# Wuziyi616/CFUN

Hardware: AMD Instinct MI355X
Metric: volumes/sec fwd+bwd, 256x256x128 8-class CT (higher is better)
Workload: dtype f32; 1 GPU; cfg2: 256x256x128 CT, stage 'finetune', 4 positive + 8 negative RoIs, U-Net b=20, 96x96x96 crops -> 192x192x192 masks, 6 losses incl. 3-D Sobel edge loss, fwd+bwd; parallelism=single GPU

## Files before the change

cfun_amd/_lib.py:

```python
import ctypes as C
import os

import torch

_HERE = os.path.dirname(os.path.abspath(__file__))
DEFAULT_LIB = os.path.join(_HERE, "libcfun_hip.so")

ACT_NONE, ACT_RELU, ACT_LRELU = 0, 1, 2
ALGO_AUTO, ALGO_DIRECT, ALGO_MFMA = 0, 1, 2
ALGO_WINO = 4
ALGO_WINO2 = 5
TILE_G16, TILE_G8 = 0x100, 0x200


class ConvParams(C.Structure):
    _fields_ = [(n, C.c_int32) for n in ("N", "Di", "Hi", "Wi", "Ci", "Do", "Ho", "Wo", "Co", "CoP", "CiP",
                                         "kd", "kh", "kw", "stride", "pd", "ph", "pw", "up2", "act")] + \
               [("slope", C.c_float)] + \
               [(n, C.c_int32) for n in ("scale_mode", "has_shift", "res_mode", "res_up2", "d2s", "d2s_cq", "tap_skip", "algo",
                                         "w_prepared")]


class ConvFusion(C.Structure):
    _fields_ = [("in_stats", C.c_void_p), ("in_act", C.c_int32), ("in_slope", C.c_float), ("out_stats", C.c_void_p),
                ("out_eps", C.c_float)]


FUSE_OUT_STATS, FUSE_IN_NORM, FUSE_IN_NORM_WGRAD = 1, 2, 4


class WeightJob(C.Structure):
    _fields_ = [("w", C.c_void_p), ("fwd", C.c_void_p), ("dgrad", C.c_void_p), ("co_idx", C.c_void_p), ("ci_idx", C.c_void_p),
                ("Co", C.c_int32), ("Ci", C.c_int32), ("T", C.c_int32), ("src_ci", C.c_int32), ("fwd_kind", C.c_int32),
                ("dgrad_kind", C.c_int32), ("block_begin", C.c_uint32), ("reserved", C.c_int32)]


WOP_NONE = 0

_P = C.c_void_p
_I = C.c_int32
_L = C.c_int64
_F = C.c_float
_Z = C.c_size_t
_PP = C.POINTER(ConvParams)
_PF = C.POINTER(ConvFusion)
# ... 213 lines not shown
```

cfun_amd/csrc/common.h:

```cpp
#pragma once
#include <hip/hip_runtime.h>
#include <stdint.h>
#include <stdlib.h>

#include "../../include/cfun_hip.h"

#define CFUN_WAVE 64

#ifdef CFUN_HIP_EMULATION
#define CFUN_DYN_LDS(T, name) T* name = reinterpret_cast<T*>(hipemu::g.dyn_lds)
#else
#define CFUN_DYN_LDS(T, name) extern __shared__ __attribute__((aligned(16))) T name[]
#endif

#define CFUN_LAUNCH_CHECK()                         \
  do {                                              \
    hipError_t e__ = hipGetLastError();             \
    if (e__ != hipSuccess) return (int)e__;         \
  } while (0)

static inline hipStream_t cfun_st(cfun_stream_t s) { return (hipStream_t)s; }

static inline size_t cfun_align_up(size_t v, size_t a) { return (v + a - 1) / a * a; }

static inline bool cfun_aligned16(const void* p) { return (((uintptr_t)p) & 15) == 0; }

struct CfunWgradDst { float* ptr; int oidhw; };

__device__ __forceinline__ float cfun_apply_act(float v, int act, float slope) {
  if (act == CFUN_ACT_RELU) return v > 0.f ? v : 0.f;
  if (act == CFUN_ACT_LRELU) return v > 0.f ? v : v * slope;
  return v;
}

__device__ __forceinline__ float cfun_fast_sqrt(float v) {
#ifdef CFUN_HIP_EMULATION
  return sqrtf(v);
#else
  return __builtin_amdgcn_sqrtf(v);
#endif
}
__device__ __forceinline__ float cfun_fast_rcp(float v) {
#ifdef CFUN_HIP_EMULATION
  return 1.0f / v;
#else
  return __builtin_amdgcn_rcpf(v);
#endif
}

__device__ __forceinline__ float cfun_fast_rsq(float v) {
#ifdef CFUN_HIP_EMULATION
  return 1.0f / sqrtf(v);
#else
  return __builtin_amdgcn_rsqf(v);
#endif
}

__device__ __forceinline__ float cfun_wave_sum(float v) {
#pragma unroll
  for (int o = 32; o > 0; o >>= 1) v += __shfl_xor(v, o, 64);
  return v;
}
__device__ __forceinline__ double cfun_wave_sum_d(double v) {
#pragma unroll
  for (int o = 32; o > 0; o >>= 1) v += __shfl_xor(v, o, 64);
  return v;
}
// ... 1 lines not shown
```

cfun_amd/csrc/conv3d.hip:

```cpp
#include <stdlib.h>

#include "conv3d_mfma.h"
#include "../../include/cfun_tile.h"

int cfun_conv_fwd_direct(const float*, const float*, const float*, const float*, const float*, float*,
                         const CfunConv3dParams*, hipStream_t);
int cfun_conv_bwd_data_direct(const float*, const float*, float*, const CfunConv3dParams*, hipStream_t);
int cfun_conv_bwd_weight_direct(const float*, const float*, CfunWgradDst, const CfunConv3dParams*, void*, size_t, hipStream_t);
size_t cfun_direct_wgrad_ws(const CfunConv3dParams*);
int cfun_wgrad_finish(const float*, CfunWgradDst, const CfunConv3dParams*, int, hipStream_t);
int cfun_wgrad_zero(CfunWgradDst, const CfunConv3dParams*, hipStream_t);
int cfun_conv_stem_supported(const CfunConv3dParams*);
int cfun_conv_stem_fwd(const float*, const float*, const float*, const float*, float*, const CfunConv3dParams*, hipStream_t);
int cfun_conv_pointwise_supported(const CfunConv3dParams*);
int cfun_conv_pointwise_in_supported(const CfunConv3dParams*);
int cfun_conv_pointwise_fwd(const float*, const float*, const float*, const float*, const float*, float*,
                            const CfunConv3dParams*, const float*, int, float, hipStream_t);
int cfun_wino_supported(const CfunConv3dParams*);
size_t cfun_wino_workspace_bytes(const CfunConv3dParams*);
int cfun_wino_s2d_dgrad_supported(const CfunConv3dParams*, const CfunConv3dParams*);
int cfun_wino_fwd(const float*, const float*, int, int, const float*, const float*, const float*, float*,
                  const CfunConv3dParams*, void*, size_t, const cfun_mfma::ConvMode*, int, hipStream_t);
int cfun_wino_is_2d(const CfunConv3dParams*);
int cfun_wino_geom(const CfunConv3dParams*);
// ... 132 lines not shown
  if (q->pd < 0 || q->ph < 0 || q->pw < 0) return false;
  q->up2 = 0; q->act = CFUN_ACT_NONE; q->scale_mode = 0; q->has_shift = 0; q->res_mode = 0; q->res_up2 = 0;
  q->d2s = 0; q->d2s_cq = 0; q->tap_skip = 0; q->w_prepared = 0;
  return true;
}

bool use_folded_s2_dgrad(const CfunConv3dParams* p) {
  return CFUN_ALGO_OF(p->algo) != CFUN_ALGO_DIRECT && p->stride == 2 && !p->up2 && !p->d2s && p->kd == 3 && p->kh == 3 && p->kw == 3 &&
         p->pd == 1 && p->ph == 1 && p->pw == 1 && !((p->Di | p->Hi | p->Wi) & 1) && !(p->Ci & 3) && !(p->Co & 3) &&
         p->Di == 2 * p->Do && p->Hi == 2 * p->Ho && p->Wi == 2 * p->Wo;
}

__global__ void __launch_bounds__(256)
k_fold_s2_dgrad_weights(const float* __restrict__ wpT, float* __restrict__ wd, int Ci, int Co, int CiP, int CoPd) {
  const int64_t total = (int64_t)8 * Co * CoPd;
  const int64_t i = (int64_t)blockIdx.x * 256 + threadIdx.x;
  if (i >= total) return;
  const int col = (int)(i % CoPd);
  const int co = (int)((i / CoPd) % Co);
  const int tap = (int)(i / ((int64_t)CoPd * Co));
  float v = 0.f;
  if (col < 8 * Ci) {
    const int q = col / Ci, ci = col - q * Ci;
    const int par[3] = {q >> 2, (q >> 1) & 1, q & 1}, off[3] = {tap >> 2, (tap >> 1) & 1, tap & 1};
    int t[3];
    bool ok = true;
    for (int d = 0; d < 3; ++d) {
      if (par[d] == 0) { t[d] = 1; ok = ok && off[d] == 0; }
      else t[d] = off[d] == 0 ? 2 : 0;
    }
    if (ok) v = wpT[((int64_t)((t[0] * 3 + t[1]) * 3 + t[2]) * Co + co) * CiP + ci];
  }
  wd[i] = v;
}

CfunConv3dParams folded_s2_params(const CfunConv3dParams* p) {
  CfunConv3dParams q = *p;
  q.Di = p->Do; q.Hi = p->Ho; q.Wi = p->Wo; q.Ci = p->Co;
  q.Do = p->Do; q.Ho = p->Ho; q.Wo = p->Wo; q.Co = 8 * p->Ci;
  q.CoP = (8 * p->Ci + 15) / 16 * 16; q.CiP = p->CoP;
  q.kd = q.kh = q.kw = 2; q.stride = 1; q.pd = q.ph = q.pw = 0;
  q.up2 = 0; q.act = CFUN_ACT_NONE; q.scale_mode = 0; q.has_shift = 0; q.res_mode = 0; q.res_up2 = 0; q.d2s = 1;
  q.d2s_cq = 0; q.tap_skip = 0; q.w_prepared = 0;
  return q;
}

int wgrad_max_nsub(const Shape* s) {
  static int cap = -1;
  if (cap < 0) {
    const char* e = getenv("CFUN_WGRAD_MAX_NSUB");
    cap = e ? atoi(e) : 5;
    if (cap < 1 || cap > 5) cap = 5;
  }
  return s->max_nsub < cap ? s->max_nsub : cap;
}

int wgrad_nsub(const CfunConv3dParams* p, const Shape* s) {
  if (p->d2s && p->tap_skip) {
    const int cqp = p->Co >> 3, mx = wgrad_max_nsub(s);
    const int tiles = (cqp + 16 * mx - 1) / (16 * mx);
    return (cqp + 16 * tiles - 1) / (16 * tiles);
  }
  return pick_nsub(p->CoP, wgrad_max_nsub(s));
}

bool use_mfma_dgrad(const CfunConv3dParams* p, CfunConv3dParams* q, const Shape** s) {
// ... 106 lines not shown
  __syncthreads();
  if (vl == 0) {
    for (int l = 1; l < lanes; ++l) {
      const int t2 = l * C4 + cg;
#pragma unroll
      for (int q = 0; q < 2; ++q)
#pragma unroll
        for (int j = 0; j < 4; ++j) acc[q][j] += sm[(t2 * 2 + q) * 4 + j];
    }
    double* out = part + ((int64_t)n * gridDim.x + blockIdx.x) * 2 * p.Co;
#pragma unroll
    for (int q = 0; q < 2; ++q)
#pragma unroll
      for (int j = 0; j < 4; ++j) out[(int64_t)q * p.Co + co + j] = acc[q][j];
  }
}

int splitk_stats_blocks(const CfunConv3dParams* p, int* lanes_out) {
  const int C4 = p->Co >> 2;
  if ((p->Co & 3) || C4 > 256 || C4 < 1) return 0;
  const int lanes = 256 / C4;
  const int64_t V = (int64_t)p->Do * p->Ho * p->Wo;
  int64_t want = (4096 + p->N - 1) / (p->N > 0 ? p->N : 1);
  int64_t maxb = (V + (int64_t)lanes * 4 - 1) / ((int64_t)lanes * 4);
  if (maxb < 1) maxb = 1;
  if (lanes_out) *lanes_out = lanes;
  return (int)(want < maxb ? want : maxb);
}

}

int cfun_splitk_stat_slots(const CfunConv3dParams* p) { return splitk_stats_blocks(p, nullptr); }

int cfun_tile_geom(const CfunConv3dParams* p, int g8_exists) {
  if (!g8_exists || (p->algo & CFUN_ALGO_TILE_G16)) return 0;
  if (p->algo & CFUN_ALGO_TILE_G8) return 1;
  if (tile_geom_knob() >= 0) return tile_geom_knob();
  return g8_exists == 1 && tile_geom_rule(p) ? 1 : 0;
}

int cfun_splitk_finish(const float* partial, int ksplit, const float* scale, const float* shift, const float* res,
                       float* y, const CfunConv3dParams* p, double* stat_part, hipStream_t st) {
  if (stat_part) {
    int lanes = 0;
    const int blocks = splitk_stats_blocks(p, &lanes);
    if (blocks <= 0) return CFUN_EINVAL;
    hipLaunchKernelGGL(k_splitk_finish_stats, dim3((unsigned)blocks, (unsigned)p->N), dim3(256), 0, st, (const float4*)partial,
                       ksplit, scale, shift, res, (float4*)y, *p, (int64_t)p->Do * p->Ho * p->Wo, lanes, stat_part);
    CFUN_LAUNCH_CHECK();
    return CFUN_OK;
  }
  const int64_t total4 = (int64_t)p->N * p->Do * p->Ho * p->Wo * (p->Co >> 2);
  int64_t blocks = (total4 + 255) / 256;
  if (blocks > 2048) blocks = 2048;
  hipLaunchKernelGGL(k_splitk_finish, dim3((unsigned)blocks), dim3(256), 0, st, (const float4*)partial, ksplit, scale, shift,
                     res, (float4*)y, *p, total4);
  CFUN_LAUNCH_CHECK();
  return CFUN_OK;
}

extern "C" {

int cfun_version(void) { return CFUN_VERSION; }

const char* cfun_error_string(int code) {
  switch (code) {
// ... 169 lines not shown
    if (!ws || !cfun_aligned16(ws) || ws_bytes < main_bytes + stat_part_bytes(p)) return CFUN_EWORKSPACE;
    fz.out_part = (double*)((char*)ws + main_bytes);
  }
  int slots = 0;
  const int rc = conv_fwd_impl(x, wp, scale, shift, res, y, p, &fz, ws, f->out_stats ? main_bytes : ws_bytes, &slots, stream);
  if (rc || !f->out_stats) return rc;
  if (slots == 0) return CFUN_EINVAL;
  const int cy = p->d2s ? (p->d2s_cq > 0 ? p->d2s_cq : (p->Co >> 3)) : p->Co;
  return cfun_stats_finalize(fz.out_part, f->out_stats, p->N, slots < 0 ? -slots : slots, cy,
                             (int64_t)p->Do * p->Ho * p->Wo * (p->d2s ? 8 : 1), f->out_eps, slots > 0, cfun_st(stream));
}

int cfun_weight_prepare_kinds(const CfunConv3dParams* p, int32_t kinds[2], size_t bytes[2]) {
  if (!kinds || !bytes) return CFUN_EINVAL;
  kinds[0] = kinds[1] = CFUN_WOP_NONE;
  bytes[0] = bytes[1] = 0;
  if (!valid_params(p)) return CFUN_EINVAL;
  const int T = p->kd * p->kh * p->kw;
  if (T > 27) return CFUN_OK;
  kinds[0] = CFUN_WOP_PACK;
  bytes[0] = (size_t)T * p->Ci * p->CoP * sizeof(float);
  const bool pointwise = CFUN_ALGO_OF(p->algo) == CFUN_ALGO_AUTO && cfun_conv_pointwise_supported(p);
  if (!pointwise && CFUN_ALGO_OF(p->algo) != CFUN_ALGO_DIRECT && mfma_shape(p) && cfun_wino_supported(p)) {
    const int twod = cfun_wino_is_2d(p);
    kinds[0] = twod ? CFUN_WOP_WINO2 : CFUN_WOP_WINO1;
    bytes[0] = (size_t)(twod ? 48 : 36) * p->Ci * p->CoP * sizeof(float);
  }
  kinds[1] = CFUN_WOP_PACKT;
  bytes[1] = (size_t)T * p->Co * p->CiP * sizeof(float);
  CfunConv3dParams q;
  const Shape* s;
  if (use_folded_s2_dgrad(p)) {
    kinds[1] = CFUN_WOP_S2FOLD;
    bytes[1] = (size_t)8 * p->Co * ((8 * p->Ci + 15) / 16 * 16) * sizeof(float);
  } else if (use_mfma_dgrad(p, &q, &s) && !p->up2 &&
             (p->d2s ? cfun_wino_s2d_dgrad_supported(p, &q) : cfun_wino_supported(&q))) {
    const int twod = cfun_wino_is_2d(&q);
    kinds[1] = twod ? CFUN_WOP_WINO2_T : CFUN_WOP_WINO1_T;
    bytes[1] = (size_t)(twod ? 48 : 36) * p->Co * p->CiP * sizeof(float);
  }
  return CFUN_OK;
}

size_t cfun_conv3d_bwd_data_workspace_bytes(const CfunConv3dParams* p) {
  if (!valid_params(p)) return 0;
  CfunConv3dParams q;
  const Shape* s;
  if (use_folded_s2_dgrad(p)) return cfun_align_up((size_t)8 * p->Co * ((8 * p->Ci + 15) / 16 * 16) * sizeof(float), 256);
  if (use_mfma_dgrad(p, &q, &s)) {
    if (p->up2) return cfun_align_up((size_t)q.N * q.Do * q.Ho * q.Wo * q.Co * sizeof(float), 256);
    ConvMode md = kPlain;
    md.flip = 1;
    if (p->d2s) { md.in_s2d = 1; md.in_cqp = p->Co >> 3; md.in_cq = p->d2s_cq > 0 ? p->d2s_cq : md.in_cqp; }
    const int nsub = pick_tile(s, q.Co, false);
    if (p->d2s) md.tap_skip = p->tap_skip ? 2 : 0;
    size_t need = (mfma_geom(&q, s, md, nsub) ? s->fwd_ws8 : s->fwd_ws)(nsub, q, md);
    if ((p->d2s ? cfun_wino_s2d_dgrad_supported(p, &q) : cfun_wino_supported(&q)) && cfun_wino_workspace_bytes(&q) > need)
      need = cfun_wino_workspace_bytes(&q);
    return cfun_align_up(need + 256, 256);
  }
  return 256;
}

int cfun_conv3d_bwd_data(const float* g, const float* wpT, float* dx, const CfunConv3dParams* p, void* ws,
                         size_t ws_bytes, cfun_stream_t stream) {
  if (!valid_params(p)) return CFUN_EINVAL;
  CfunConv3dParams q;
  const Shape* s;
  const bool prepared = (p->w_prepared & 2) != 0;
  if (use_folded_s2_dgrad(p)) {
    if (!cfun_aligned16(g) || !cfun_aligned16(wpT) || !cfun_aligned16(dx) || !cfun_aligned16(ws)) return CFUN_EALIGN;
    if (ws_bytes < cfun_conv3d_bwd_data_workspace_bytes(p)) return CFUN_EWORKSPACE;
    q = folded_s2_params(p);
    const float* wd = wpT;
    if (!prepared) {
      const int64_t nw = (int64_t)8 * p->Co * q.CoP;
      hipLaunchKernelGGL(k_fold_s2_dgrad_weights, dim3((unsigned)((nw + 255) / 256)), dim3(256), 0, cfun_st(stream), wpT,
                         (float*)ws, p->Ci, p->Co, p->CiP, q.CoP);
      CFUN_LAUNCH_CHECK();
      wd = (const float*)ws;
    }
    const Shape* s2 = find_shape(2, 2, 2, 1);
    const int nsub = pick_nsub(q.Co, s2->max_nsub);
    return (mfma_geom(&q, s2, kPlain, nsub) ? s2->fwd8 : s2->fwd)(nsub, g, wd, nullptr, nullptr, nullptr, dx, q, kPlain, nullptr, 0,
                                                                   cfun_st(stream));
  }
  if (use_mfma_dgrad(p, &q, &s)) {
    if (!cfun_aligned16(g) || !cfun_aligned16(wpT) || !cfun_aligned16(dx)) return CFUN_EALIGN;
    const int nsub = pick_tile(s, q.Co, false);
    ConvMode md = kPlain;
    md.flip = 1;
    if (p->d2s) {
      md.in_s2d = 1;
      md.in_cqp = p->Co >> 3;
      md.in_cq = p->d2s_cq > 0 ? p->d2s_cq : md.in_cqp;
      md.tap_skip = p->tap_skip ? 2 : 0;
    }
    const bool wino = !p->up2 && (p->d2s ? cfun_wino_s2d_dgrad_supported(p, &q) : cfun_wino_supported(&q));
    if (wino && cfun_aligned16(ws) && ws_bytes >= cfun_wino_workspace_bytes(&q))
      return cfun_wino_fwd(g, wpT, 1, p->d2s ? (p->Co >> 3) : 0, nullptr, nullptr, nullptr, dx, &q, ws, ws_bytes, nullptr,
                           prepared, cfun_st(stream));
    if (wino && prepared) return CFUN_EWORKSPACE;
    const FwdFn fwd = mfma_geom(&q, s, md, nsub) ? s->fwd8 : s->fwd;
    if (!p->up2) return fwd(nsub, g, wpT, nullptr, nullptr, nullptr, dx, q, md, ws, cfun_aligned16(ws) ? ws_bytes : 0, cfun_st(stream));
    if (ws_bytes < cfun_conv3d_bwd_data_workspace_bytes(p) || !cfun_aligned16(ws)) return CFUN_EWORKSPACE;
    const int rc = fwd(nsub, g, wpT, nullptr, nullptr, nullptr, (float*)ws, q, md, nullptr, 0, cfun_st(stream));
    if (rc) return rc;
    return cfun_upsample2_bwd((const float*)ws, dx, p->N, p->Di, p->Hi, p->Wi, p->Ci, stream);
  }
  return cfun_conv_bwd_data_direct(g, wpT, dx, p, cfun_st(stream));
}

static bool wgrad_mfma_fits(const CfunConv3dParams* p) {
  const int64_t lim = (int64_t)1 << 31;
  const int64_t go = (int64_t)p->N * p->Do * p->Ho * p->Wo * p->Co;
  return (int64_t)p->N * p->Di * p->Hi * p->Wi * p->Ci < lim && go < lim;
}

// ... 100 lines not shown
```

cfun_amd/csrc/conv3d_mfma.h:

```cpp
#pragma once
#include <type_traits>

#include "common.h"

typedef float f32x4 __attribute__((ext_vector_type(4)));

int cfun_splitk_finish(const float* partial, int ksplit, const float* scale, const float* shift, const float* res,
                       float* y, const CfunConv3dParams* p, double* stat_part, hipStream_t st);
int cfun_splitk_stat_slots(const CfunConv3dParams* p);

namespace cfun_mfma {

constexpr int pad_plane(int v, int rs, int g = 0) { return rs != 1 ? (v | 1) : v + (((g ? 8 : 16) - (v % 32)) + 32) % 32; }
constexpr int pad_row16(int v) { return (v % 32 == 16) ? v : v + 16; }
constexpr int cdiv(int a, int b) { return (a + b - 1) / b; }
constexpr int row_stride(int nt) { return nt <= 16 ? 16 : nt <= 48 ? 48 : nt <= 80 ? 80 : pad_row16((nt + 15) / 16 * 16); }

__device__ __forceinline__ unsigned xcd_remap(unsigned bid, unsigned nwg) {
  const unsigned q = nwg >> 3, r = nwg & 7u, xcd = bid & 7u, local = bid >> 3;
  const unsigned base = xcd < r ? xcd * (q + 1) : r * (q + 1) + (xcd - r) * q;
  return base + local;
}

__device__ __forceinline__ void tile_raster(unsigned t, int ntz, int nty, int ntx, int& tz, int& ty, int& tx) {
// ... 492 lines not shown

template <int KD, int KH, int KW, int S>
constexpr bool has_rem_tiles() {
  return (KD == 3 && KH == 3 && KW == 3) || (KD == 1 && KH == 1 && KW == 1 && S == 1);
}

template <int KD, int KH, int KW, int S>
constexpr int max_nsub() { return KD * KH * KW > 27 ? 1 : 5; }

template <int KD, int KH, int KW, int S, int G = 0>
int dispatch_nsub(int nsub, const float* x, const float* wp, const float* scale, const float* shift, const float* res,
                  float* y, const CfunConv3dParams& p, const ConvMode& flip, void* ws, size_t wsb, hipStream_t st) {
  if constexpr (has_rem_tiles<KD, KH, KW, S>()) {
    if (nsub == 1 + 8 * 1) return launch_conv_mfma<KD, KH, KW, S, 1, 1, G>(x, wp, scale, shift, res, y, p, flip, ws, wsb, st);
    if constexpr (G == 0)
      if (nsub == 2 + 8 * 2) return launch_conv_mfma<KD, KH, KW, S, 2, 2>(x, wp, scale, shift, res, y, p, flip, ws, wsb, st);
    if (nsub == 0 + 8 * 2) return launch_conv_mfma<KD, KH, KW, S, 0, 2, G>(x, wp, scale, shift, res, y, p, flip, ws, wsb, st);
  }
  if (nsub >= 8 || nsub < 1) return CFUN_EINVAL;
  if constexpr (max_nsub<KD, KH, KW, S>() == 1) {
    if (nsub != 1) return CFUN_EINVAL;
    return launch_conv_mfma<KD, KH, KW, S, 1, 0, G>(x, wp, scale, shift, res, y, p, flip, ws, wsb, st);
  } else {
    switch (nsub) {
      case 1: return launch_conv_mfma<KD, KH, KW, S, 1, 0, G>(x, wp, scale, shift, res, y, p, flip, ws, wsb, st);
      case 2: return launch_conv_mfma<KD, KH, KW, S, 2, 0, G>(x, wp, scale, shift, res, y, p, flip, ws, wsb, st);
      case 3: return launch_conv_mfma<KD, KH, KW, S, 3, 0, G>(x, wp, scale, shift, res, y, p, flip, ws, wsb, st);
      case 4: return launch_conv_mfma<KD, KH, KW, S, 4, 0, G>(x, wp, scale, shift, res, y, p, flip, ws, wsb, st);
      default: return launch_conv_mfma<KD, KH, KW, S, 5, 0, G>(x, wp, scale, shift, res, y, p, flip, ws, wsb, st);
    }
  }
}

struct WgIn {
  const float* stats;
  int act;
  float slope;
};

template <int KD, int KH, int KW, int S, int G = 0>
struct WgTile {
  static constexpr int TD = (S == 1) ? 2 : 1, TH = G ? 8 : 4, TW = G ? 8 : 16;
  static constexpr int XQ = TW / 4;
  static constexpr int TVOX = TD * TH * TW;
  static constexpr int TAPS = KD * KH * KW;
  static constexpr bool COMPACT = TAPS == 1;
  static constexpr int RS = COMPACT ? 1 : S;
  static constexpr int IZ = COMPACT ? TD : (TD - 1) * S + KD;
  static constexpr int IY = COMPACT ? TH : (TH - 1) * S + KH;
  static constexpr int IX = COMPACT ? TW : (TW - 1) * S + KW;
  static constexpr int IVOX = IZ * IY * IX;
  static constexpr int XS = 16;
  static constexpr int X_LOADS = cdiv(IVOX * 4, 256);
  static constexpr int TSPLIT = TAPS >= 4 ? 4 : 1;
  static constexpr int KSPLIT = 4 / TSPLIT;
  static constexpr int TPW = cdiv(TAPS, TSPLIT);
};

template <int KD, int KH, int KW, int S, int NSUB, bool TSKIP, int PACK, bool IN, int G>
__device__ __forceinline__ void
wgrad_body(float* smem, const float* __restrict__ x, const float* __restrict__ g, float* __restrict__ partial,
           const CfunConv3dParams& p, int ntz, int nty, int ntx, int cot, int cis, int chunk, int tiles_per_chunk,
           int ntiles, const WgIn& fin) {
  using T = WgTile<KD, KH, KW, S, G>;
  constexpr int TAPS = T::TAPS, NT = 16 * NSUB, GS = pad_row16(NT);
  constexpr int NLIVE = TSKIP ? 8 : TAPS;
// ... 521 lines not shown
    return cfun_mfma::dispatch_nsub<KD, KH, KW, S>(nsub, x, wp, scale, shift, res, y, p, flip, ws, wsb, st);        \
  }                                                                                                                 \
  size_t cfun_mfma_fwd_ws_##NAME(int nsub, const CfunConv3dParams& p, const cfun_mfma::ConvMode& md) {              \
    return cfun_mfma::fwd_workspace<KD, KH, KW, S>(nsub, p, md);                                                    \
  }                                                                                                                 \
  void cfun_mfma_wgrad_plan_##NAME(const CfunConv3dParams& p, int nsub, cfun_mfma::WgPlan* w) {                     \
    *w = cfun_mfma::wgrad_plan<KD, KH, KW, S>(p, nsub);                                                             \
  }                                                                                                                 \
  int cfun_mfma_wgrad_##NAME(const float* x, const float* g, float* partial, const CfunConv3dParams& p,             \
                             const cfun_mfma::WgPlan& w, hipStream_t st) {                                          \
    return cfun_mfma::dispatch_wgrad<KD, KH, KW, S>(x, g, partial, p, w, st);                                       \
  }

#define CFUN_MFMA_DECL_G8(NAME)                                                                                     \
  int cfun_mfma_fwd_g8_##NAME(int nsub, const float* x, const float* wp, const float* scale, const float* shift,    \
                              const float* res, float* y, const CfunConv3dParams& p,                                \
                              const cfun_mfma::ConvMode& flip, void* ws, size_t wsb, hipStream_t st);               \
  size_t cfun_mfma_fwd_ws_g8_##NAME(int nsub, const CfunConv3dParams& p, const cfun_mfma::ConvMode& md);

#define CFUN_MFMA_DEFINE_G8(NAME, KD, KH, KW, S)                                                                    \
  int cfun_mfma_fwd_g8_##NAME(int nsub, const float* x, const float* wp, const float* scale, const float* shift,    \
                              const float* res, float* y, const CfunConv3dParams& p,                                \
                              const cfun_mfma::ConvMode& flip, void* ws, size_t wsb, hipStream_t st) {              \
    return cfun_mfma::dispatch_nsub<KD, KH, KW, S, 1>(nsub, x, wp, scale, shift, res, y, p, flip, ws, wsb, st);     \
  }                                                                                                                 \
  size_t cfun_mfma_fwd_ws_g8_##NAME(int nsub, const CfunConv3dParams& p, const cfun_mfma::ConvMode& md) {           \
    return cfun_mfma::fwd_workspace<KD, KH, KW, S, 1>(nsub, p, md);                                                 \
  }

CFUN_MFMA_DECL_G8(k333s1)
CFUN_MFMA_DECL_G8(k333s2)
CFUN_MFMA_DECL_G8(k222s1)

#define CFUN_WGRAD_DECL_G8(NAME)                                                                                    \
  void cfun_mfma_wgrad_plan_g8_##NAME(const CfunConv3dParams& p, int nsub, cfun_mfma::WgPlan* w);                   \
  int cfun_mfma_wgrad_g8_##NAME(const float* x, const float* g, float* partial, const CfunConv3dParams& p,          \
                                const cfun_mfma::WgPlan& w, hipStream_t st);

#define CFUN_WGRAD_DEFINE_G8(NAME, KD, KH, KW, S)                                                                   \
  void cfun_mfma_wgrad_plan_g8_##NAME(const CfunConv3dParams& p, int nsub, cfun_mfma::WgPlan* w) {                  \
    *w = cfun_mfma::wgrad_plan<KD, KH, KW, S, 1>(p, nsub);                                                          \
  }                                                                                                                 \
  int cfun_mfma_wgrad_g8_##NAME(const float* x, const float* g, float* partial, const CfunConv3dParams& p,          \
                                const cfun_mfma::WgPlan& w, hipStream_t st) {                                       \
    return cfun_mfma::dispatch_wgrad<KD, KH, KW, S, 1>(x, g, partial, p, w, st);                                    \
  }

CFUN_WGRAD_DECL_G8(k333s1)
CFUN_WGRAD_DECL_G8(k333s2)
CFUN_WGRAD_DECL_G8(k111s1)

int cfun_tile_geom(const CfunConv3dParams* p, int g8_exists);

CFUN_MFMA_DECL(k333s1)
CFUN_MFMA_DECL(k333s2)
CFUN_MFMA_DECL(k111s1)
CFUN_MFMA_DECL(k111s2)
CFUN_MFMA_DECL(k133s1)
CFUN_MFMA_DECL(k311s1)
CFUN_MFMA_DECL(k555s1)
CFUN_MFMA_DECL(k222s1)
```

cfun_amd/csrc/conv3d_mfma_k222s1.hip:

```cpp
#include "conv3d_mfma.h"

CFUN_MFMA_DEFINE(k222s1, 2, 2, 2, 1)
```

cfun_amd/csrc/conv3d_mfma_k222s1_g8.hip:

```cpp
#include "conv3d_mfma.h"

CFUN_MFMA_DEFINE_G8(k222s1, 2, 2, 2, 1)
```

cfun_amd/csrc/weight_prep.hip:

```cpp
#include "common.h"

namespace {

constexpr int kBlock = 256;
constexpr int TS = 28;

__device__ __forceinline__ float4 wino_row(float g0, float g1, float g2) {
  return make_float4(g0, 0.5f * ((g0 + g2) + g1), 0.5f * ((g0 + g2) - g1), g2);
}

__global__ void __launch_bounds__(kBlock)
k_weight_prepare(const CfunWeightJob* __restrict__ jobs, int njobs) {
  __shared__ float s[16 * 16 * TS];
  __shared__ int sj;
  const int tid = threadIdx.x;
  if (tid == 0) {
    int j = 0;
    while (j + 1 < njobs && jobs[j + 1].block_begin <= blockIdx.x) ++j;
    sj = j;
  }
  __syncthreads();
  const CfunWeightJob J = jobs[sj];
  const int local = (int)(blockIdx.x - J.block_begin);
  const int tiles_ci = (J.Ci + 15) >> 4;
  const int co0 = (local / tiles_ci) * 16, ci0 = (local % tiles_ci) * 16;
  const int T = J.T, Co = J.Co, Ci = J.Ci;
  const int CoP = (Co + 15) & ~15, CiP = (Ci + 15) & ~15;

  for (int i = tid; i < 16 * 16 * T; i += kBlock) {
    const int co = i / (16 * T), r = i - co * 16 * T, ci = r / T, t = r - ci * T;
    const int gco = co0 + co, gci = ci0 + ci;
    float v = 0.f;
    if (gco < Co && gci < Ci) {
      const int64_t sco = J.co_idx ? J.co_idx[gco] : gco, sci = J.ci_idx ? J.ci_idx[gci] : gci;
      v = J.w[(sco * J.src_ci + sci) * T + t];
    }
    s[(co * 16 + ci) * TS + t] = v;
  }
  __syncthreads();

  if (J.fwd_kind == CFUN_WOP_PACK) {
    for (int i = tid; i < 256 * T; i += kBlock) {
      const int t = i >> 8, ci = (i >> 4) & 15, co = i & 15;
      if (ci0 + ci < Ci) J.fwd[((int64_t)t * Ci + ci0 + ci) * CoP + co0 + co] = s[(co * 16 + ci) * TS + t];
    }
// ... 17 lines not shown
      u[base] = wino_row(t[0].x, t[1].x, t[2].x);
      u[base + step] = wino_row(t[0].y, t[1].y, t[2].y);
      u[base + 2 * step] = wino_row(t[0].z, t[1].z, t[2].z);
      u[base + 3 * step] = wino_row(t[0].w, t[1].w, t[2].w);
    }
  }

  if (J.dgrad_kind == CFUN_WOP_PACKT) {
    for (int i = tid; i < 256 * T; i += kBlock) {
      const int t = i >> 8, co = (i >> 4) & 15, ci = i & 15;
      if (co0 + co < Co) J.dgrad[((int64_t)t * Co + co0 + co) * CiP + ci0 + ci] = s[(co * 16 + ci) * TS + t];
    }
  } else if (J.dgrad_kind == CFUN_WOP_WINO1_T) {
    float4* u = reinterpret_cast<float4*>(J.dgrad);
    for (int i = tid; i < 256 * 9; i += kBlock) {
      const int r9 = i >> 8, co = (i >> 4) & 15, ci = i & 15;
      const float* g = s + (co * 16 + ci) * TS + 26 - r9 * 3;
      if (co0 + co < Co) u[((int64_t)r9 * Co + co0 + co) * CiP + ci0 + ci] = wino_row(g[0], g[-1], g[-2]);
    }
  } else if (J.dgrad_kind == CFUN_WOP_WINO2_T) {
    float4* u = reinterpret_cast<float4*>(J.dgrad);
    for (int i = tid; i < 256 * 3; i += kBlock) {
      const int dz = i >> 8, co = (i >> 4) & 15, ci = i & 15;
      if (co0 + co >= Co) continue;
      const float* g = s + (co * 16 + ci) * TS + 26 - dz * 9;
      float4 t[3];
#pragma unroll
      for (int kx = 0; kx < 3; ++kx) t[kx] = wino_row(g[-kx], g[-3 - kx], g[-6 - kx]);
      const int64_t base = ((int64_t)(dz * 4) * Co + co0 + co) * CiP + ci0 + ci, step = (int64_t)Co * CiP;
      u[base] = wino_row(t[0].x, t[1].x, t[2].x);
      u[base + step] = wino_row(t[0].y, t[1].y, t[2].y);
      u[base + 2 * step] = wino_row(t[0].z, t[1].z, t[2].z);
      u[base + 3 * step] = wino_row(t[0].w, t[1].w, t[2].w);
    }
  } else if (J.dgrad_kind == CFUN_WOP_S2FOLD) {
    const int CoPd = (8 * Ci + 15) & ~15;
    for (int i = tid; i < 256 * 64; i += kBlock) {
      const int e = i >> 8, co = (i >> 4) & 15, ci = i & 15;
      if (co0 + co >= Co || ci0 + ci >= Ci) continue;
      const int tap = e >> 3, q = e & 7;
      const int par[3] = {q >> 2, (q >> 1) & 1, q & 1}, off[3] = {tap >> 2, (tap >> 1) & 1, tap & 1};
      int t[3];
      bool ok = true;
#pragma unroll
      for (int d = 0; d < 3; ++d) {
        if (par[d] == 0) { t[d] = 1; ok = ok && off[d] == 0; }
        else t[d] = off[d] == 0 ? 2 : 0;
      }
      J.dgrad[((int64_t)tap * Co + co0 + co) * CoPd + q * Ci + ci0 + ci] = ok ? s[(co * 16 + ci) * TS + (t[0] * 3 + t[1]) * 3 + t[2]] : 0.f;
    }
    if (ci0 == 0)
      for (int i = tid; i < 8 * 16 * 16; i += kBlock) {
        const int tap = i >> 8, co = (i >> 4) & 15, col = 8 * Ci + (i & 15);
        if (co0 + co < Co && col < CoPd) J.dgrad[((int64_t)tap * Co + co0 + co) * CoPd + col] = 0.f;
      }
  }
}


__device__ __forceinline__ int fold_a(int p, int t, int k) { return ((p + t - (k >> 1)) >> 1) + 1; }

__global__ void __launch_bounds__(256)
k_fold_up2_fwd(const float* __restrict__ w, float* __restrict__ wf, int Co, int Ci, int k, int cqp, int64_t total) {
  for (int64_t idx = (int64_t)blockIdx.x * 256 + threadIdx.x; idx < total; idx += (int64_t)gridDim.x * 256) {
    int64_t r = idx;
    const int abc = (int)(r % 27); r /= 27;
// ... 56 lines not shown
    if (wino && J.T != 27) return CFUN_EINVAL;
    if (total > 0x7fffffffLL) return CFUN_EINVAL;
    J.block_begin = (uint32_t)total;
    total += (int64_t)((J.Co + 15) / 16) * ((J.Ci + 15) / 16);
  }
  if (total > 0x7fffffffLL) return CFUN_EINVAL;
  *nblocks = total;
  return CFUN_OK;
}

int cfun_fold_up2_fwd(const float* w, float* wf, int32_t Co, int32_t Ci, int32_t k, int32_t cqp, cfun_stream_t stream) {
  if (!w || !wf || Co <= 0 || Ci <= 0 || (k != 3 && k != 5) || cqp < Co) return CFUN_EINVAL;
  const int64_t total = (int64_t)8 * cqp * Ci * 27;
  int64_t blocks = (total + 255) / 256;
  if (blocks > 256 * 64) blocks = 256 * 64;
  hipLaunchKernelGGL(k_fold_up2_fwd, dim3((unsigned)blocks), dim3(256), 0, cfun_st(stream), w, wf, Co, Ci, k, cqp, total);
  CFUN_LAUNCH_CHECK();
  return CFUN_OK;
}

int cfun_fold_up2_bwd(const float* g, float* dw, int32_t Co, int32_t Ci, int32_t k, int32_t cqp, cfun_stream_t stream) {
  if (!g || !dw || Co <= 0 || Ci <= 0 || (k != 3 && k != 5) || cqp < Co) return CFUN_EINVAL;
  const int64_t total = (int64_t)Co * Ci * k * k * k;
  int64_t blocks = (total + 255) / 256;
  if (blocks > 256 * 64) blocks = 256 * 64;
  hipLaunchKernelGGL(k_fold_up2_bwd, dim3((unsigned)blocks), dim3(256), 0, cfun_st(stream), g, dw, Co, Ci, k, cqp, total);
  CFUN_LAUNCH_CHECK();
  return CFUN_OK;
}

int cfun_weight_prepare(const CfunWeightJob* jobs_dev, int32_t njobs, int64_t nblocks, cfun_stream_t stream) {
  if (njobs <= 0 || nblocks <= 0) return CFUN_OK;
  if (!jobs_dev || nblocks > 0x7fffffffLL) return CFUN_EINVAL;
  hipLaunchKernelGGL(k_weight_prepare, dim3((unsigned)nblocks), dim3(kBlock), 0, cfun_st(stream), jobs_dev, njobs);
  CFUN_LAUNCH_CHECK();
  return CFUN_OK;
}

}
```

include/cfun_hip.h:

```cpp
#ifndef CFUN_HIP_H
#define CFUN_HIP_H

#include <stddef.h>
#include <stdint.h>

#ifdef __cplusplus
extern "C" {
#endif

typedef void* cfun_stream_t;

#define CFUN_VERSION 100
#define CFUN_OK 0
#define CFUN_EINVAL (-1)
#define CFUN_EWORKSPACE (-2)
#define CFUN_EALIGN (-3)

#define CFUN_ACT_NONE 0
#define CFUN_ACT_RELU 1
#define CFUN_ACT_LRELU 2

#define CFUN_ALGO_AUTO 0
#define CFUN_ALGO_DIRECT 1
#define CFUN_ALGO_MFMA 2
#define CFUN_ALGO_WINO 4
#define CFUN_ALGO_WINO2 5
#define CFUN_ALGO_TILE_G16 0x100
#define CFUN_ALGO_TILE_G8 0x200
#define CFUN_ALGO_OF(algo) ((algo) & 0xff)

int cfun_version(void);
const char* cfun_error_string(int code);

typedef struct CfunConv3dParams {
  int32_t N;
  int32_t Di, Hi, Wi, Ci;
  int32_t Do, Ho, Wo, Co;
  int32_t CoP, CiP;
  int32_t kd, kh, kw;
  int32_t stride;
  int32_t pd, ph, pw;
  int32_t up2;
  int32_t act;
  float slope;
  int32_t scale_mode;
  int32_t has_shift;
  int32_t res_mode;
  int32_t res_up2;
  int32_t d2s;
  int32_t d2s_cq;
  int32_t tap_skip;
  int32_t algo;
  int32_t w_prepared;
} CfunConv3dParams;

size_t cfun_conv3d_fwd_workspace_bytes(const CfunConv3dParams* p);
#define CFUN_KERNEL_DIRECT 0
#define CFUN_KERNEL_MFMA 1
#define CFUN_KERNEL_WINO 2
#define CFUN_KERNEL_STEM 3
#define CFUN_KERNEL_POINTWISE 4
// ... 200 lines not shown
```

Measured before the change: 26.35 volumes/s.

## Skip structurally-zero taps in folded stride-2 conv data-gradient

Replaces the dense folded stride-2 dgrad, a 2x2x2 conv producing 8 parity outputs from zero-padded weights, with a dedicated MFMA kernel. It stores only the 27 live tap/parity weight blocks and skips the zero taps per parity group. The work is split across two block halves, each owning four parity groups, and the results are scattered directly into the upsampled dx layout. Weight preparation emits the compact layout, and the dense path stays available through an env knob or an algo flag. This cuts wasted MFMA work on zeros (27 of 64 blocks are live), at the cost of a new kernel with more accumulators and different tiling that could hurt occupancy.

```diff
diff --git a/cfun_amd/_lib.py b/cfun_amd/_lib.py
--- a/cfun_amd/_lib.py
+++ b/cfun_amd/_lib.py
@@ -11,6 +11,7 @@
 ALGO_WINO = 4
 ALGO_WINO2 = 5
 TILE_G16, TILE_G8 = 0x100, 0x200
+S2_DENSE = 0x400
 
 
 class ConvParams(C.Structure):
diff --git a/cfun_amd/csrc/common.h b/cfun_amd/csrc/common.h
--- a/cfun_amd/csrc/common.h
+++ b/cfun_amd/csrc/common.h
@@ -33,6 +33,38 @@
   return v;
 }
 
+#define CFUN_S2_LIVE_BLOCKS 27
+__host__ __device__ constexpr int cfun_s2_group_parity(int gs) { return (int)((0x46532107u >> (4 * gs)) & 7u); }
+__host__ __device__ constexpr int cfun_s2_group_taps(int gs) {
+  const int q = cfun_s2_group_parity(gs);
+  return 1 << ((q & 1) + ((q >> 1) & 1) + (q >> 2));
+}
+__host__ __device__ constexpr int cfun_s2_group_base(int gs) {
+  int b = 0;
+  for (int g = 0; g < gs; ++g) b += cfun_s2_group_taps(g);
+  return b;
+}
+__host__ __device__ constexpr int cfun_s2_tap_rank(int q, int tap) {
+  int r = 0, k = 0;
+  for (int d = 0; d < 3; ++d)
+    if ((q >> d) & 1) { r |= ((tap >> d) & 1) << k; ++k; }
+  return r;
+}
+__host__ __device__ inline void cfun_s2_block_decode(int blk, int* q_out, int* tap_out) {
+  int gs = 0;
+  while (gs < 7 && blk >= cfun_s2_group_base(gs + 1)) ++gs;
+  const int q = cfun_s2_group_parity(gs);
+  int r = blk - cfun_s2_group_base(gs), tap = 0;
+  for (int d = 0; d < 3; ++d)
+    if ((q >> d) & 1) { tap |= (r & 1) << d; r >>= 1; }
+  *q_out = q; *tap_out = tap;
+}
+__host__ __device__ constexpr int cfun_s2_source_tap(int q, int tap) {
+  int t = 0;
+  for (int d = 2; d >= 0; --d) t = t * 3 + (((q >> d) & 1) ? (((tap >> d) & 1) ? 0 : 2) : 1);
+  return t;
+}
+
 __device__ __forceinline__ float cfun_fast_sqrt(float v) {
 #ifdef CFUN_HIP_EMULATION
   return sqrtf(v);
diff --git a/cfun_amd/csrc/conv3d.hip b/cfun_amd/csrc/conv3d.hip
--- a/cfun_amd/csrc/conv3d.hip
+++ b/cfun_amd/csrc/conv3d.hip
@@ -188,6 +188,31 @@
     if (ok) v = wpT[((int64_t)((t[0] * 3 + t[1]) * 3 + t[2]) * Co + co) * CiP + ci];
   }
   wd[i] = v;
+}
+
+__global__ void __launch_bounds__(256)
+k_fold_s2_dgrad_live(const float* __restrict__ wpT, float* __restrict__ wd, int Ci, int Co, int CiP, int cqp) {
+  const int64_t total = (int64_t)CFUN_S2_LIVE_BLOCKS * Co * cqp;
+  const int64_t i = (int64_t)blockIdx.x * 256 + threadIdx.x;
+  if (i >= total) return;
+  const int ci = (int)(i % cqp);
+  const int co = (int)((i / cqp) % Co);
+  int q, tap;
+  cfun_s2_block_decode((int)(i / ((int64_t)cqp * Co)), &q, &tap);
+  wd[i] = ci < Ci ? wpT[((int64_t)cfun_s2_source_tap(q, tap) * Co + co) * CiP + ci] : 0.f;
+}
+
+int s2_dense_knob() {
+  static int v = -1;
+  if (v < 0) { const char* e = getenv("CFUN_S2_DGRAD_DENSE"); v = (e && atoi(e) == 1) ? 1 : 0; }
+  return v;
+}
+int s2_dgrad_ns(const CfunConv3dParams* p) { return (p->Ci > 16 && p->Ci <= 32) ? 2 : 1; }
+bool s2_dgrad_dense(const CfunConv3dParams* p) { return s2_dense_knob() || (p->algo & CFUN_ALGO_S2_DENSE); }
+
+size_t s2_operand_bytes(const CfunConv3dParams* p, bool dense) {
+  if (dense) return (size_t)8 * p->Co * ((8 * p->Ci + 15) / 16 * 16) * sizeof(float);
+  return (size_t)CFUN_S2_LIVE_BLOCKS * p->Co * ((p->Ci + 15) / 16 * 16) * sizeof(float);
 }
 
 CfunConv3dParams folded_s2_params(const CfunConv3dParams* p) {
@@ -360,6 +385,8 @@
 
 int cfun_splitk_stat_slots(const CfunConv3dParams* p) { return splitk_stats_blocks(p, nullptr); }
 
+int cfun_s2_dgrad_dense_knob() { return s2_dense_knob(); }
+
 int cfun_tile_geom(const CfunConv3dParams* p, int g8_exists) {
   if (!g8_exists || (p->algo & CFUN_ALGO_TILE_G16)) return 0;
   if (p->algo & CFUN_ALGO_TILE_G8) return 1;
@@ -595,7 +622,7 @@
   const Shape* s;
   if (use_folded_s2_dgrad(p)) {
     kinds[1] = CFUN_WOP_S2FOLD;
-    bytes[1] = (size_t)8 * p->Co * ((8 * p->Ci + 15) / 16 * 16) * sizeof(float);
+    bytes[1] = s2_operand_bytes(p, s2_dense_knob());
   } else if (use_mfma_dgrad(p, &q, &s) && !p->up2 &&
              (p->d2s ? cfun_wino_s2d_dgrad_supported(p, &q) : cfun_wino_supported(&q))) {
     const int twod = cfun_wino_is_2d(&q);
@@ -609,7 +636,7 @@
   if (!valid_params(p)) return 0;
   CfunConv3dParams q;
   const Shape* s;
-  if (use_folded_s2_dgrad(p)) return cfun_align_up((size_t)8 * p->Co * ((8 * p->Ci + 15) / 16 * 16) * sizeof(float), 256);
+  if (use_folded_s2_dgrad(p)) return cfun_align_up(s2_operand_bytes(p, s2_dgrad_dense(p)), 256);
   if (use_mfma_dgrad(p, &q, &s)) {
     if (p->up2) return cfun_align_up((size_t)q.N * q.Do * q.Ho * q.Wo * q.Co * sizeof(float), 256);
     ConvMode md = kPlain;
@@ -635,18 +662,26 @@
     if (!cfun_aligned16(g) || !cfun_aligned16(wpT) || !cfun_aligned16(dx) || !cfun_aligned16(ws)) return CFUN_EALIGN;
     if (ws_bytes < cfun_conv3d_bwd_data_workspace_bytes(p)) return CFUN_EWORKSPACE;
     q = folded_s2_params(p);
+    const bool dense = s2_dgrad_dense(p);
+    if (prepared && dense && !s2_dense_knob()) return CFUN_EINVAL;
     const float* wd = wpT;
     if (!prepared) {
-      const int64_t nw = (int64_t)8 * p->Co * q.CoP;
-      hipLaunchKernelGGL(k_fold_s2_dgrad_weights, dim3((unsigned)((nw + 255) / 256)), dim3(256), 0, cfun_st(stream), wpT,
-                         (float*)ws, p->Ci, p->Co, p->CiP, q.CoP);
+      const int cqp = (p->Ci + 15) / 16 * 16;
+      const int64_t nw = dense ? (int64_t)8 * p->Co * q.CoP : (int64_t)CFUN_S2_LIVE_BLOCKS * p->Co * cqp;
+      if (dense)
+        hipLaunchKernelGGL(k_fold_s2_dgrad_weights, dim3((unsigned)((nw + 255) / 256)), dim3(256), 0, cfun_st(stream), wpT,
+                           (float*)ws, p->Ci, p->Co, p->CiP, q.CoP);
+      else
+        hipLaunchKernelGGL(k_fold_s2_dgrad_live, dim3((unsigned)((nw + 255) / 256)), dim3(256), 0, cfun_st(stream), wpT,
+                           (float*)ws, p->Ci, p->Co, p->CiP, cqp);
       CFUN_LAUNCH_CHECK();
       wd = (const float*)ws;
     }
     const Shape* s2 = find_shape(2, 2, 2, 1);
     const int nsub = pick_nsub(q.Co, s2->max_nsub);
-    return (mfma_geom(&q, s2, kPlain, nsub) ? s2->fwd8 : s2->fwd)(nsub, g, wd, nullptr, nullptr, nullptr, dx, q, kPlain, nullptr, 0,
-                                                                   cfun_st(stream));
+    const int geom = mfma_geom(&q, s2, kPlain, nsub);
+    if (!dense) return (geom ? cfun_mfma_s2_dgrad_skip_g8 : cfun_mfma_s2_dgrad_skip)(s2_dgrad_ns(p), g, wd, dx, *p, cfun_st(stream));
+    return (geom ? s2->fwd8 : s2->fwd)(nsub, g, wd, nullptr, nullptr, nullptr, dx, q, kPlain, nullptr, 0, cfun_st(stream));
   }
   if (use_mfma_dgrad(p, &q, &s)) {
     if (!cfun_aligned16(g) || !cfun_aligned16(wpT) || !cfun_aligned16(dx)) return CFUN_EALIGN;
diff --git a/cfun_amd/csrc/conv3d_mfma.h b/cfun_amd/csrc/conv3d_mfma.h
--- a/cfun_amd/csrc/conv3d_mfma.h
+++ b/cfun_amd/csrc/conv3d_mfma.h
@@ -548,6 +548,169 @@
   }
 }
 
+template <int NS, int G, int HALF>
+__device__ __forceinline__ void
+s2_dgrad_skip_body(float* smem, const float* __restrict__ g, const float* __restrict__ wd, float* __restrict__ dx, int n, int z0,
+                   int y0, int x0, int rng, int Do, int Ho, int Wo, int Kc, int Ci, int cqp) {
+  using T = FwdTile<2, 2, 2, 1, G>;
+  constexpr int NB = HALF ? 14 : 13, B0 = HALF ? 13 : 0;
+  static_assert(cfun_s2_group_base(4) == 13 && cfun_s2_group_base(8) == CFUN_S2_LIVE_BLOCKS, "halves of the live-block operand");
+  constexpr int NT = 16 * NS, NTP = row_stride(NT);
+  constexpr int W_ITEMS = NB * NT;
+  constexpr int W_LOADS = cdiv(W_ITEMS, 256);
+  float* Xl = smem;
+  float* Wl = smem + 4 * T::PLANEP;
+  const int tid = threadIdx.x, lane = tid & 63, wv = __builtin_amdgcn_readfirstlane(tid >> 6);
+
+  int64_t in_off[T::IN_LOADS];
+#pragma unroll
+  for (int i = 0; i < T::IN_LOADS; ++i) {
+    const int idx = tid + i * T::PASS;
+    in_off[i] = -1;
+    if (tid < T::PASS && idx < T::IVOX) {
+      const int vx = x0 + idx % T::IX, vy = y0 + (idx / T::IX) % T::IY, vz = z0 + idx / (T::IX * T::IY);
+      if (vz < Do && vy < Ho && vx < Wo) in_off[i] = ((((int64_t)n * Do + vz) * Ho + vy) * Wo + vx) * Kc;
+    }
+  }
+  const int xl0 = T::IXS == T::IX ? tid : (tid / T::IX) * T::IXS + tid % T::IX;
+  const int col0 = rng * NT;
+  float4 xin[T::IN_LOADS], win[W_LOADS];
+  auto prefetch = [&](int c) {
+#pragma unroll
+    for (int i = 0; i < T::IN_LOADS; ++i)
+      xin[i] = in_off[i] >= 0 ? *reinterpret_cast<const float4*>(g + in_off[i] + c * 4) : make_float4(0.f, 0.f, 0.f, 0.f);
+#pragma unroll
+    for (int i = 0; i < W_LOADS; ++i) {
+      const int it = tid + i * 256;
+      win[i] = make_float4(0.f, 0.f, 0.f, 0.f);
+      if (it < W_ITEMS) {
+        const int row = it / (NT / 4), col = col0 + (it % (NT / 4)) * 4;
+        if (col < cqp) win[i] = *reinterpret_cast<const float4*>(wd + ((int64_t)(B0 + (row >> 2)) * Kc + c * 4 + (row & 3)) * cqp + col);
+      }
+    }
+  };
+  auto commit = [&]() {
+#pragma unroll
+    for (int i = 0; i < T::IN_LOADS; ++i) {
+      const int idx = tid + i * T::PASS;
+      if (tid < T::PASS && idx < T::IVOX) {
+        const int l = T::IXS == T::IX ? idx : xl0 + i * (T::PASS / T::IX) * T::IXS;
+        Xl[l] = xin[i].x; Xl[T::PLANEP + l] = xin[i].y;
+        Xl[2 * T::PLANEP + l] = xin[i].z; Xl[3 * T::PLANEP + l] = xin[i].w;
+      }
+    }
+#pragma unroll
+    for (int i = 0; i < W_LOADS; ++i) {
+      const int it = tid + i * 256;
+      if (it < W_ITEMS) *reinterpret_cast<float4*>(Wl + (it / (NT / 4)) * NTP + (it % (NT / 4)) * 4) = win[i];
+    }
+  };
+
+  f32x4 acc[4][4][NS];
+#pragma unroll
+  for (int gi = 0; gi < 4; ++gi)
+#pragma unroll
+    for (int m = 0; m < 4; ++m)
+#pragma unroll
+      for (int nn = 0; nn < NS; ++nn) acc[gi][m][nn] = f32x4{0.f, 0.f, 0.f, 0.f};
+
+  const int mrow = (lane & 15) / T::TW, mx = (lane & 15) % T::TW;
+  const float* Xw = Xl + (lane >> 4) * T::PLANEP + (wv * T::IY + mrow) * T::IXS + mx;
+  const float* Ww = Wl + (lane >> 4) * NTP + (lane & 15);
+  auto mfma_chunk = [&]() {
+#pragma unroll
+    for (int tap = 0; tap < 8; ++tap) {
+      const int dz = tap >> 2, dy = (tap >> 1) & 1, dxo = tap & 1;
+      float b[4];
+#pragma unroll
+      for (int m = 0; m < 4; ++m) b[m] = Xw[(dz * T::IY + (m * T::MR + dy)) * T::IXS + dxo];
+#pragma unroll
+      for (int gi = 0; gi < 4; ++gi) {
+        const int q = cfun_s2_group_parity(HALF * 4 + gi);
+        if (tap & ~q & 7) continue;
+        const int blk = cfun_s2_group_base(HALF * 4 + gi) - B0 + cfun_s2_tap_rank(q, tap);
+#pragma unroll
+        for (int nn = 0; nn < NS; ++nn) {
+          const float a = Ww[blk * 4 * NTP + nn * 16];
+#pragma unroll
+          for (int m = 0; m < 4; ++m) acc[gi][m][nn] = __builtin_amdgcn_mfma_f32_16x16x4f32(a, b[m], acc[gi][m][nn], 0, 0, 0);
+        }
+      }
+    }
+  };
+
+  const int nchunks = Kc >> 2;
+  if (nchunks > 0) prefetch(0);
+  for (int c = 0; c < nchunks; ++c) {
+    __syncthreads();
+    commit();
+    __syncthreads();
+    if (c + 1 < nchunks) prefetch(c + 1);
+    mfma_chunk();
+  }
+
+  const int oz = z0 + wv, ox = x0 + mx;
+  if (oz >= Do || ox >= Wo) return;
+#pragma unroll
+  for (int gi = 0; gi < 4; ++gi) {
+    const int q = cfun_s2_group_parity(HALF * 4 + gi);
+#pragma unroll
+    for (int nn = 0; nn < NS; ++nn) {
+      const int oc = col0 + nn * 16 + (lane >> 4) * 4;
+      if (oc >= Ci) continue;
+#pragma unroll
+      for (int m = 0; m < 4; ++m) {
+        const int oy = y0 + m * T::MR + mrow;
+        if (oy >= Ho) continue;
+        const int64_t hv = (((int64_t)n * 2 * Do + 2 * oz + (q >> 2)) * 2 * Ho + 2 * oy + ((q >> 1) & 1)) * 2 * Wo + 2 * ox + (q & 1);
+        const f32x4& a4 = acc[gi][m][nn];
+        *reinterpret_cast<float4*>(dx + hv * Ci + oc) = make_float4(a4[0], a4[1], a4[2], a4[3]);
+      }
+    }
+  }
+}
+
+template <int NS, int G>
+__global__ void __launch_bounds__(256, 2)
+k_s2_dgrad_skip(const float* __restrict__ g, const float* __restrict__ wd, float* __restrict__ dx, int Do, int Ho, int Wo,
+                int Kc, int Ci, int cqp, int ntz, int nty, int ntx, int nrange) {
+  using T = FwdTile<2, 2, 2, 1, G>;
+  CFUN_DYN_LDS(float, smem);
+  unsigned lid = xcd_remap(blockIdx.x, gridDim.x);
+  const int half = lid & 1u; lid >>= 1;
+  const int rng = lid % nrange; lid /= nrange;
+  const unsigned per_n = (unsigned)(ntz * nty * ntx);
+  const int n = lid / per_n;
+  int tz, ty, tx;
+  tile_raster(lid - (unsigned)n * per_n, ntz, nty, ntx, tz, ty, tx);
+  if (half == 0) s2_dgrad_skip_body<NS, G, 0>(smem, g, wd, dx, n, tz * T::TD, ty * T::TH, tx * T::TW, rng, Do, Ho, Wo, Kc, Ci, cqp);
+  else s2_dgrad_skip_body<NS, G, 1>(smem, g, wd, dx, n, tz * T::TD, ty * T::TH, tx * T::TW, rng, Do, Ho, Wo, Kc, Ci, cqp);
+}
+
+template <int NS, int G>
+int launch_s2_dgrad_skip(const float* g, const float* wd, float* dx, const CfunConv3dParams& p, hipStream_t st) {
+  using T = FwdTile<2, 2, 2, 1, G>;
+  constexpr int NTP = row_stride(16 * NS);
+  const int cqp = (p.Ci + 15) / 16 * 16;
+  if ((cqp / 16) % NS) return CFUN_EINVAL;
+  const int ntz = cdiv(p.Do, T::TD), nty = cdiv(p.Ho, T::TH), ntx = cdiv(p.Wo, T::TW), nrange = cqp / 16 / NS;
+  const int64_t nblk = (int64_t)p.N * ntz * nty * ntx * nrange * 2;
+  if (nblk == 0) return CFUN_OK;
+  if (nblk > 0x7fffffffLL) return CFUN_EINVAL;
+  const size_t lds = (size_t)(4 * T::PLANEP + 14 * 4 * NTP) * sizeof(float);
+  hipLaunchKernelGGL((k_s2_dgrad_skip<NS, G>), dim3((unsigned)nblk), dim3(256), lds, st, g, wd, dx, p.Do, p.Ho, p.Wo, p.Co, p.Ci,
+                     cqp, ntz, nty, ntx, nrange);
+  CFUN_LAUNCH_CHECK();
+  return CFUN_OK;
+}
+
+template <int G>
+int dispatch_s2_dgrad_skip(int ns, const float* g, const float* wd, float* dx, const CfunConv3dParams& p, hipStream_t st) {
+  if (ns == 1) return launch_s2_dgrad_skip<1, G>(g, wd, dx, p, st);
+  if (ns == 2) return launch_s2_dgrad_skip<2, G>(g, wd, dx, p, st);
+  return CFUN_EINVAL;
+}
+
 struct WgIn {
   const float* stats;
   int act;
@@ -1135,6 +1298,9 @@
 CFUN_MFMA_DECL_G8(k333s2)
 CFUN_MFMA_DECL_G8(k222s1)
 
+int cfun_mfma_s2_dgrad_skip(int ns, const float* g, const float* wd, float* dx, const CfunConv3dParams& p, hipStream_t st);
+int cfun_mfma_s2_dgrad_skip_g8(int ns, const float* g, const float* wd, float* dx, const CfunConv3dParams& p, hipStream_t st);
+
 #define CFUN_WGRAD_DECL_G8(NAME)                                                                                    \
   void cfun_mfma_wgrad_plan_g8_##NAME(const CfunConv3dParams& p, int nsub, cfun_mfma::WgPlan* w);                   \
   int cfun_mfma_wgrad_g8_##NAME(const float* x, const float* g, float* partial, const CfunConv3dParams& p,          \
diff --git a/cfun_amd/csrc/conv3d_mfma_k222s1.hip b/cfun_amd/csrc/conv3d_mfma_k222s1.hip
--- a/cfun_amd/csrc/conv3d_mfma_k222s1.hip
+++ b/cfun_amd/csrc/conv3d_mfma_k222s1.hip
@@ -1,3 +1,7 @@
 #include "conv3d_mfma.h"
 
 CFUN_MFMA_DEFINE(k222s1, 2, 2, 2, 1)
+
+int cfun_mfma_s2_dgrad_skip(int ns, const float* g, const float* wd, float* dx, const CfunConv3dParams& p, hipStream_t st) {
+  return cfun_mfma::dispatch_s2_dgrad_skip<0>(ns, g, wd, dx, p, st);
+}
diff --git a/cfun_amd/csrc/conv3d_mfma_k222s1_g8.hip b/cfun_amd/csrc/conv3d_mfma_k222s1_g8.hip
--- a/cfun_amd/csrc/conv3d_mfma_k222s1_g8.hip
+++ b/cfun_amd/csrc/conv3d_mfma_k222s1_g8.hip
@@ -1,3 +1,7 @@
 #include "conv3d_mfma.h"
 
 CFUN_MFMA_DEFINE_G8(k222s1, 2, 2, 2, 1)
+
+int cfun_mfma_s2_dgrad_skip_g8(int ns, const float* g, const float* wd, float* dx, const CfunConv3dParams& p, hipStream_t st) {
+  return cfun_mfma::dispatch_s2_dgrad_skip<1>(ns, g, wd, dx, p, st);
+}
diff --git a/cfun_amd/csrc/weight_prep.hip b/cfun_amd/csrc/weight_prep.hip
--- a/cfun_amd/csrc/weight_prep.hip
+++ b/cfun_amd/csrc/weight_prep.hip
@@ -1,4 +1,6 @@
 #include "common.h"
+
+int cfun_s2_dgrad_dense_knob();
 
 namespace {
 
@@ -10,7 +12,7 @@
 }
 
 __global__ void __launch_bounds__(kBlock)
-k_weight_prepare(const CfunWeightJob* __restrict__ jobs, int njobs) {
+k_weight_prepare(const CfunWeightJob* __restrict__ jobs, int njobs, int s2_dense) {
   __shared__ float s[16 * 16 * TS];
   __shared__ int sj;
   const int tid = threadIdx.x;
@@ -94,6 +96,15 @@
       u[base + step] = wino_row(t[0].y, t[1].y, t[2].y);
       u[base + 2 * step] = wino_row(t[0].z, t[1].z, t[2].z);
       u[base + 3 * step] = wino_row(t[0].w, t[1].w, t[2].w);
+    }
+  } else if (J.dgrad_kind == CFUN_WOP_S2FOLD && !s2_dense) {
+    const int cqp = CiP;
+    for (int i = tid; i < 256 * CFUN_S2_LIVE_BLOCKS; i += kBlock) {
+      const int blk = i >> 8, co = (i >> 4) & 15, ci = i & 15;
+      if (co0 + co >= Co) continue;
+      int q, tap;
+      cfun_s2_block_decode(blk, &q, &tap);
+      J.dgrad[((int64_t)blk * Co + co0 + co) * cqp + ci0 + ci] = ci0 + ci < Ci ? s[(co * 16 + ci) * TS + cfun_s2_source_tap(q, tap)] : 0.f;
     }
   } else if (J.dgrad_kind == CFUN_WOP_S2FOLD) {
     const int CoPd = (8 * Ci + 15) & ~15;
@@ -216,7 +227,8 @@
 int cfun_weight_prepare(const CfunWeightJob* jobs_dev, int32_t njobs, int64_t nblocks, cfun_stream_t stream) {
   if (njobs <= 0 || nblocks <= 0) return CFUN_OK;
   if (!jobs_dev || nblocks > 0x7fffffffLL) return CFUN_EINVAL;
-  hipLaunchKernelGGL(k_weight_prepare, dim3((unsigned)nblocks), dim3(kBlock), 0, cfun_st(stream), jobs_dev, njobs);
+  hipLaunchKernelGGL(k_weight_prepare, dim3((unsigned)nblocks), dim3(kBlock), 0, cfun_st(stream), jobs_dev, njobs,
+                     cfun_s2_dgrad_dense_knob());
   CFUN_LAUNCH_CHECK();
   return CFUN_OK;
 }
diff --git a/include/cfun_hip.h b/include/cfun_hip.h
--- a/include/cfun_hip.h
+++ b/include/cfun_hip.h
@@ -27,6 +27,7 @@
 #define CFUN_ALGO_WINO2 5
 #define CFUN_ALGO_TILE_G16 0x100
 #define CFUN_ALGO_TILE_G8 0x200
+#define CFUN_ALGO_S2_DENSE 0x400
 #define CFUN_ALGO_OF(algo) ((algo) & 0xff)
 
 int cfun_version(void);
```

After: 26.56 volumes/s (median of 6 runs). About the same (+0.8%).
